# PINTO0309/human-instance-segmentation

Measured on AMD Instinct MI355X. Metric: ROI-masks/sec (fwd) + train step/s, B0 640×480×8-ROI, 1/2/4/8 MI355X, higher is better.
Workload: dtype bf16; 1 GPU; C2: B0 inference 640x480, batch 32/GPU x 8 ROIs/img, ROI 64x48, mask 128x96; global_batch=32, parallelism=dp1 (images sharded, model replicated, no collective), schedule=2-stream pipeline (UNet of step k+1 overlaps head of step k)

## Files before the change

human-instance-segmentation_amd/csrc/misc.hip:

```cpp
#include <float.h>
#include "common.h"
#include "gfx950_prims.h"
#include "head2.h"

namespace hiseg {

static inline unsigned nblocks(long long n, int bs) { return (unsigned)((n + bs - 1) / bs); }

template <typename T>
__global__ void __launch_bounds__(256) maxpool2x2_kernel(const void* in, int N, int H, int W, int C, void* out) {
  constexpr int K = Chunk<T>::N;
  const int nch = C / K;
  const int Ho = H / 2, Wo = W / 2;
  const long long gid = (long long)blockIdx.x * 256 + threadIdx.x;
  const long long total = (long long)N * Ho * Wo * nch;
  if (gid >= total) return;
  const int ch = (int)(gid % nch);
  long long p = gid / nch;
  const int x = (int)(p % Wo); p /= Wo;
  const int y = (int)(p % Ho);
  const int n = (int)(p / Ho);
  const uint4* src = reinterpret_cast<const uint4*>(in);
  float m[K], v[K];
  for (int e = 0; e < K; ++e) m[e] = -FLT_MAX;
#pragma unroll
  for (int dy = 0; dy < 2; ++dy)
#pragma unroll
    for (int dx = 0; dx < 2; ++dx) {
      const long long pix = ((long long)n * H + 2 * y + dy) * W + 2 * x + dx;
      Chunk<T>::unpack(src[pix * nch + ch], v);
#pragma unroll
      for (int e = 0; e < K; ++e) m[e] = fmaxf(m[e], v[e]);
    }
  reinterpret_cast<uint4*>(out)[gid] = Chunk<T>::pack(m);
}
// ... 276 lines not shown
  if (v2) hipLaunchKernelGGL(se_gate_out_kernel<true>, g2, dim3(256), lds, s, partial, splits, C, b1, Cr, act, beta, w2, b2, gate);
  else hipLaunchKernelGGL(se_gate_out_kernel<false>, g2, dim3(256), lds, s, partial, splits, C, b1, Cr, act, beta, w2, b2, gate);
}

static bool se2_enabled() {
  const char* e = getenv("HISEG_SE2");
  return !(e && atoi(e) == 0);
}

static void se_mlp(const float* w1, const float* b1, int Cr, const float* w2, const float* b2, int act, float beta, int N,
                   int HW, int C, float* scratch, float* gate, hipStream_t s) {
  hipLaunchKernelGGL(se_hidden_kernel, dim3(N, (Cr + 3) / 4), dim3(256), 0, s, gate, HW, C, w1, b1, Cr, act, beta, scratch);
  hipLaunchKernelGGL(se_out_kernel, dim3(N, (C + 3) / 4), dim3(256), 0, s, scratch, C, Cr, w2, b2, gate);
}

template <typename T>
__global__ void __launch_bounds__(256) channel_scale_kernel(const void* x, int N, long long HW, int C, const float* gate,
                                                            void* out) {
  constexpr int K = Chunk<T>::N;
  const int nch = C / K;
  const long long gid = (long long)blockIdx.x * 256 + threadIdx.x;
  const long long total = (long long)N * HW * nch;
  if (gid >= total) return;
  const int ch = (int)(gid % nch);
  const long long n = gid / nch / HW;
  float v[K];
  Chunk<T>::unpack(reinterpret_cast<const uint4*>(x)[gid], v);
  const float* g = gate + n * C + ch * K;
#pragma unroll
  for (int e = 0; e < K; ++e) v[e] *= g[e];
  reinterpret_cast<uint4*>(out)[gid] = Chunk<T>::pack(v);
}

constexpr int kDwXS = 4;

template <typename T, int KS, int ST>
__global__ void __launch_bounds__(256) dwconv_kernel(const void* in, int H, int W, int C, const float* w,
                                                     const float* scale, const float* shift, int act, void* out,
                                                     int Ho, int Wo, float* gap) {
  constexpr int V = Chunk<T>::N;
  constexpr int NIN = (kDwXS - 1) * ST + KS;
  __shared__ float red[256 * V];
  const int nch = C / V;
  const int g0 = blockIdx.z * 256;
  const int CT = (nch - g0) < 256 ? (nch - g0) : 256;
  const int R = 256 / CT;
  const int t = threadIdx.x;
  const int cl = t % CT, r = t / CT;
  const int ch = g0 + cl;
  const bool live = r < R;
  const int n = blockIdx.y, tiles = gridDim.x, tile = blockIdx.x;
  const int sx = (Wo + kDwXS - 1) / kDwXS;
  const int strips = Ho * sx;
  const int s0 = (int)((long long)strips * tile / tiles), s1 = (int)((long long)strips * (tile + 1) / tiles);
  const int c = ch * V;
  const int pad = KS / 2;
  float sc[V], sh[V], gs[V];
#pragma unroll
  for (int e = 0; e < V; ++e) { sc[e] = scale[c + e]; sh[e] = shift[c + e]; gs[e] = 0.f; }
  const uint4* src = reinterpret_cast<const uint4*>(in) + (long long)n * H * W * nch;
  uint4* dst = reinterpret_cast<uint4*>(out) + (long long)n * Ho * Wo * nch;
  if (live) {
    for (int st = s0 + r; st < s1; st += R) {
      const int oy = st / sx;
      const int ox0 = (st - oy * sx) * kDwXS;
      float acc[kDwXS][V];
#pragma unroll
// ... 137 lines not shown
            if (kx < 0 || kx >= KS) continue;
#pragma unroll
            for (int e = 0; e < 4; ++e) acc[xo][e] += wk[ky * KS + kx][e] * v[e];
          }
        }
      }
#pragma unroll
      for (int xo = 0; xo < kDwXS; ++xo) {
        if (ox0 + xo >= Wo) break;
        float o[4];
#pragma unroll
        for (int e = 0; e < 4; ++e) {
          o[e] = apply_act(acc[xo][e] * sc[e] + sh[e], act);
          gs[e] += o[e];
        }
        dst[((long long)oy * Wo + ox0 + xo) * nq + q] = make_uint2(f2bf2(o[0], o[1]), f2bf2(o[2], o[3]));
      }
    }
  }
  if (gap == nullptr) return;
#pragma unroll
  for (int e = 0; e < 4; ++e) red[t * 4 + e] = gs[e];
  __syncthreads();
  if (r == 0 && live) {
    for (int rr = 1; rr < R; ++rr)
#pragma unroll
      for (int e = 0; e < 4; ++e) gs[e] += red[(rr * CT + cl) * 4 + e];
    float* gp = gap + ((long long)n * tiles + tile) * C + c;
#pragma unroll
    for (int e = 0; e < 4; ++e) gp[e] = gs[e];
  }
}

constexpr int kDwTH = 8, kDwTW = 16, kDwCG = 64, kDwPS = kDwCG * 2 + 8;
template <int KS, int ST, bool ZP = false, int CP = 4>
__global__ void __launch_bounds__(256) dwconv_t_kernel(const void* in, int H, int W, int C, const float* w,
                                                       const float* scale, const float* shift, int act, void* out,
                                                       int Ho, int Wo, float* gap, int xcd) {
  constexpr int IH = (kDwTH - 1) * ST + KS, IW = (kDwTW - 1) * ST + KS;
  constexpr int NIN = (kDwXS - 1) * ST + KS;
  constexpr int NSTRIP = kDwTH * (kDwTW / kDwXS);
  extern __shared__ __attribute__((aligned(16))) char dws[];
  const int t = threadIdx.x;
  int bt = blockIdx.x, n = blockIdx.y, gz = blockIdx.z;
  if (xcd) {
    const int nwg = gridDim.x * gridDim.y * gridDim.z;
    const int orig = blockIdx.x + gridDim.x * (blockIdx.y + gridDim.y * blockIdx.z);
    int wg = xcd_major(orig, nwg);
    if (xcd == 2) {
      gz = wg % gridDim.z;
      wg /= gridDim.z;
      bt = wg % gridDim.x;
      n = wg / gridDim.x;
    } else {
      bt = wg % gridDim.x;
      wg /= gridDim.x;
      n = wg % gridDim.y;
      gz = wg / gridDim.y;
    }
  }
  const int g0 = gz * kDwCG;
  const int ntx = (Wo + kDwTW - 1) / kDwTW;
  const int ty = bt / ntx, tx = bt - ty * ntx;
  const int oy0 = ty * kDwTH, ox0 = tx * kDwTW;
  const int iy0 = oy0 * ST - KS / 2, ix0 = ox0 * ST - KS / 2;
  const int nch = C >> 3;
  const uint4* src = reinterpret_cast<const uint4*>(in) + (long long)n * H * W * nch;
// ... 499 lines not shown
}

extern "C" int hiseg_dw_gap_tiles(int N, int Ho, int Wo) {
  const int strips = Ho * ((Wo + kDwXS - 1) / kDwXS);
  int t = 2048 / (N > 0 ? N : 1);
  if (t < 1) t = 1;
  int by_len = strips / 2;
  if (by_len < 1) by_len = 1;
  return t < by_len ? t : by_len;
}

static bool dw_q_enabled() {
  const char* e = getenv("HISEG_DWCONV_Q");
  return !(e && atoi(e) == 0);
}

static bool dw_use_tiles(int dtype, int C, int K, int stride) {
  const char* e = getenv("HISEG_DWCONV_T");
  const int m = e ? atoi(e) : 1;
  if (dtype != HISEG_BF16 || m == 0 || !dw_q_enabled()) return false;
  return m == 2 || (C < 2048 && ((stride == 1 && C >= 64) || (K == 5 && C >= 192)));
}

extern "C" int hiseg_dw_gap_parts(int dtype, int N, int Ho, int Wo, int C, int K, int stride) {
  if (dw_use_tiles(dtype, C, K, stride)) return ((Ho + kDwTH - 1) / kDwTH) * ((Wo + kDwTW - 1) / kDwTW);
  return hiseg_dw_gap_tiles(N, Ho, Wo);
}

static size_t dw_lds(int KS, int ST) {
  const size_t win = (size_t)((kDwTH - 1) * ST + KS) * ((kDwTW - 1) * ST + KS) * kDwPS;
  return win > 256 * 4 * sizeof(float) ? win : 256 * 4 * sizeof(float);
}

static int dw_xcd_remap() {
  const char* e = getenv("HISEG_DWCONV_XCD");
  return e ? atoi(e) : 2;
}

static bool dw_zero_pad_q(int K, int stride) {
  const char* e = getenv("HISEG_DWCONV_QZP");
  return !(e && e[0] == '0') && (K == 3 || stride == 2);
}

static int dw_xcd_remap_q() {
  const char* e = getenv("HISEG_DWCONV_QXCD");
  return e ? atoi(e) : 2;
}

template <int KS, int ST>
static void dw_t_attr() {
  static bool done = false;
  if (!done) {
    (void)hipFuncSetAttribute((const void*)dwconv_t_kernel<KS, ST, false>, hipFuncAttributeMaxDynamicSharedMemorySize,
                              (int)dw_lds(KS, ST));
    (void)hipFuncSetAttribute((const void*)dwconv_t_kernel<KS, ST, true>, hipFuncAttributeMaxDynamicSharedMemorySize,
                              (int)dw_lds(KS, ST));
    (void)hipFuncSetAttribute((const void*)dwconv_t_kernel<KS, ST, false, 2>,
                              hipFuncAttributeMaxDynamicSharedMemorySize, (int)dw_lds(KS, ST));
    (void)hipFuncSetAttribute((const void*)dwconv_t_kernel<KS, ST, true, 2>, hipFuncAttributeMaxDynamicSharedMemorySize,
                              (int)dw_lds(KS, ST));
    done = true;
  }
}

static bool dw_zero_pad(int K) {
  const char* e = getenv("HISEG_DWCONV_ZP");
  const int m = e ? atoi(e) : 2;
  return m == 2 || (K == 3 && m == 1);
}

static int dw_cp(int K, int C) {
  const char* e = getenv("HISEG_DWCONV_CP");
  const int m = e ? atoi(e) : 0;
  return m == 2 || m == 4 ? m : (K == 5 || C < 512 ? 2 : 4);
}

static int dwconv_launch(int dtype, const void* in, int N, int H, int W, int C, int K, int stride, const float* w,
                         const float* scale, const float* shift, int act, void* out, int Ho, int Wo, float* gap,
                         hipStream_t s) {
  HISEG_REQUIRE(in && w && scale && shift && out && N > 0 && H > 0 && W > 0, HISEG_ERR_BAD_ARG, "dwconv: bad args");
  HISEG_REQUIRE(act != HISEG_ACT_SWISH, HISEG_ERR_BAD_ARG, "dwconv: Swish(beta) is not an EfficientNet activation");
  HISEG_REQUIRE(C % chunk_of(dtype) == 0, HISEG_ERR_BAD_SHAPE, "dwconv: C must be chunk aligned");
  HISEG_REQUIRE((K == 3 || K == 5) && (stride == 1 || stride == 2), HISEG_ERR_BAD_SHAPE, "dwconv: K %d stride %d", K,
                stride);
  HISEG_REQUIRE(Ho == (H + 2 * (K / 2) - K) / stride + 1 && Wo == (W + 2 * (K / 2) - K) / stride + 1, HISEG_ERR_BAD_SHAPE,
                "dwconv: output grid mismatch");
  HISEG_REQUIRE((reinterpret_cast<uintptr_t>(w) & 15) == 0 && (long long)H * W * C < (1ll << 31), HISEG_ERR_BAD_SHAPE,
                "dwconv: weights must be 16-B aligned, image < 2^31 elements");
  const int nch = C / chunk_of(dtype);
  const int nq = C / 4, ctq = dw_quads_per_block(nq);
  const int tiles = hiseg_dw_gap_tiles(N, Ho, Wo);
  dim3 grid(tiles, N, (nch + 255) / 256);
  dim3 gridq(tiles, N, (nq + ctq - 1) / ctq);
  const bool dwq = dw_q_enabled();
  const bool dwt = dw_use_tiles(dtype, C, K, stride);
  const int tiles2 = ((Ho + kDwTH - 1) / kDwTH) * ((Wo + kDwTW - 1) / kDwTW);
  const dim3 gridt(tiles2, N, (C + kDwCG - 1) / kDwCG);
#define DW_L(KS, ST)                                                                                          \
  do {                                                                                                        \
    if (dtype == HISEG_BF16 && dwt) {                                                                         \
      dw_t_attr<KS, ST>();                                                                                    \
      const bool zp = dw_zero_pad(KS), cp2 = dw_cp(KS, C) == 2;                                                    \
      if (zp && cp2)                                                                                          \
        hipLaunchKernelGGL((dwconv_t_kernel<KS, ST, true, 2>), gridt, dim3(256), dw_lds(KS, ST), s, in, H, W, \
// ... 268 lines not shown
```

human-instance-segmentation_amd/hiseg/_lib.py:

```python
from __future__ import annotations

import contextlib
import ctypes
import os

import torch

_HERE = os.path.dirname(os.path.abspath(__file__))
LIB_PATH = os.environ.get("HISEG_LIB", os.path.join(_HERE, "libhiseg.so"))

HISEG_F32 = 0
HISEG_BF16 = 1
HISEG_POST_F32, HISEG_POST_F16, HISEG_POST_F32_TO_F16 = 0, 2, 3
ACT_NONE, ACT_RELU, ACT_SIGMOID, ACT_SILU, ACT_GELU, ACT_SWISH = 0, 1, 2, 3, 4, 5


class ActCode(int):

    def __new__(cls, code: int, beta: float = 1.0):
        o = int.__new__(cls, code)
        o.beta = float(beta)
        return o

    def __repr__(self):
# ... 235 lines not shown
        "hiseg_xcd_major": ([c_int, c_int], c_int),
        "hiseg_xcd_major_fill": ([c_int, c_int, c_int, P], c_int),
        "hiseg_stream_create_cu_mask": ([ctypes.POINTER(ctypes.c_uint), c_int, ctypes.POINTER(c_void_p)], c_int),
        "hiseg_stream_destroy": ([P], c_int),
        "hiseg_comm_load": ([ctypes.c_char_p], c_int),
        "hiseg_comm_unique_id": ([P], c_int),
        "hiseg_comm_init": ([ctypes.POINTER(c_void_p), c_int, P, c_int, c_int], c_int),
        "hiseg_comm_all_reduce": ([P, P, c_ll, c_int, c_int, P], c_int),
        "hiseg_comm_destroy": ([P], c_int),
        "hiseg_roi_align_fwd": ([ctypes.POINTER(RoiAlignDesc), P], c_int),
        "hiseg_conv2d_fwd": ([ctypes.POINTER(Conv2dDesc), P], c_int),
        "hiseg_conv2d_fwd_variant": ([ctypes.POINTER(Conv2dDesc), c_int, P], c_int),
        "hiseg_conv2d_workspace_bytes": ([ctypes.POINTER(Conv2dDesc)], c_ll),
        "hiseg_conv2d_last_path": ([], c_int),
        "hiseg_conv2d_path_stats": ([ctypes.POINTER(c_ll), c_int, c_int], c_int),
        "hiseg_maxpool2x2_fwd": ([c_int, P, c_int, c_int, c_int, c_int, P, P], c_int),
        "hiseg_attn_spatial_fwd": ([c_int, P, c_int, c_int, c_int, c_int, P, c_int, P, P, P, P], c_int),
        "hiseg_attn_map_fwd": ([c_int, P, c_int, c_int, c_int, c_int, P, c_int, P, P, P], c_int),
        "hiseg_pixel_scale_fwd": ([c_int, P, c_ll, c_int, P, P, P], c_int),
        "hiseg_conv2d_fused_ok": ([ctypes.POINTER(Conv2dDesc)], c_int),
        "hiseg_resblock_fused_ok": ([ctypes.POINTER(Conv2dDesc), ctypes.POINTER(Conv2dDesc)], c_int),
        "hiseg_resblock_fwd": ([ctypes.POINTER(Conv2dDesc), ctypes.POINTER(Conv2dDesc), P], c_int),
        "hiseg_hier_combine_tn_fwd": ([P, c_int, c_int, c_int, P, P, P, P, c_int, c_float, c_int, P, P, P, P, P, P],
                                      c_int),
        "hiseg_gap_splits": ([c_int], c_int),
        "hiseg_se_gate_fwd": ([c_int, P, c_int, c_int, c_int, P, P, c_int, P, P, c_int, c_float, P, P, P], c_int),
        "hiseg_channel_scale_fwd": ([c_int, P, c_int, c_int, c_int, P, P, P], c_int),
        "hiseg_dwconv_fwd": ([c_int, P, c_int, c_int, c_int, c_int, c_int, c_int, P, P, P, c_int, P,
                              c_int, c_int, P], c_int),
        "hiseg_dw_gap_tiles": ([c_int, c_int, c_int], c_int),
        "hiseg_dw_gap_parts": ([c_int, c_int, c_int, c_int, c_int, c_int, c_int], c_int),
        "hiseg_dwconv_gap_fwd": ([c_int, P, c_int, c_int, c_int, c_int, c_int, c_int, P, P, P, c_int, P,
                                  c_int, c_int, P, P], c_int),
        "hiseg_se_gate_partials_fwd": ([P, c_int, c_int, c_int, c_int, P, P, c_int, P, P, c_int, P, P], c_int),
        "hiseg_image_max_fwd": ([P, c_ll, P, P], c_int),
        "hiseg_input_norm_fwd": ([c_int, P, c_int, c_int, c_int, c_int, P, P, P, P, c_int, P], c_int),
        "hiseg_hier_combine_fwd": ([c_int, P, c_int, c_int, c_int, P, c_int, P, P, P, c_int, c_float, c_int, P, P,
                                    P, P, P, P, P, P], c_int),
        "hiseg_ubf_ln_tables": ([P, c_int, c_int, c_int, P, P, P, P, c_float, c_int, P, P, P, P, P], c_int),
        "hiseg_nhwc_to_nchw_fwd": ([c_int, P, c_int, c_int, c_int, c_int, c_int, c_int, P, P], c_int),
        "hiseg_nchw_to_nhwc_fwd": ([c_int, P, c_int, c_int, c_int, c_int, P, c_int, P], c_int),
        "hiseg_instance_masks_fwd": ([P, c_int, c_int, c_int, c_int, P, P], c_int),
        "hiseg_binary_masks_fwd": ([c_int, P, c_int, c_int, c_int, c_int, P, P, P, P], c_int),
        "hiseg_resize_bilinear_fwd": ([P, c_int, c_int, c_int, P, c_int, c_int, P], c_int),
        "hiseg_distance_mask_fwd": ([P, c_ll, P, P, P], c_int),
        "hiseg_output_conv_fwd": ([P, c_int, c_int, c_int, P, P, P, P], c_int),
        "hiseg_conv2d_wgrad_dims": ([ctypes.POINTER(Conv2dDesc), c_int, P, P, P], c_int),
        "hiseg_conv2d_wgrad": ([ctypes.POINTER(Conv2dDesc), P, c_int, c_int, c_int, P, c_int, P], c_int),
        "hiseg_wgrad_path_stats": ([ctypes.POINTER(c_ll), c_int], c_int),
        "hiseg_struct_sizes": ([ctypes.POINTER(c_ll), c_int], c_int),
        "hiseg_conv2d_stats_tiles": ([ctypes.POINTER(Conv2dDesc)], c_int),
        "hiseg_bn_finalize_n": ([P, c_int, c_int, c_ll, P, P, c_float, c_float, P, P, P, P, P, P, P], c_int),
        "hiseg_wgrad_last_path": ([], c_int),
        "hiseg_conv2d_wgrad_reduce": ([P, c_int, ctypes.POINTER(WgradMap), P, P, c_int, P], c_int),
        "hiseg_pack_weights": ([P, c_int, c_int, P], c_int),
        "hiseg_bn_partials": ([], c_int),
        "hiseg_bn_last_path": ([], c_int),
        "hiseg_bn_stats": ([c_int, P, c_ll, c_int, c_int, c_int, P, P], c_int),
        "hiseg_bn_finalize": ([P, c_int, c_ll, P, P, c_float, c_float, P, P, P, P, P, P, P], c_int),
        "hiseg_bn_apply": ([ctypes.POINTER(BnApplyDesc), P], c_int),
        "hiseg_bn_bwd": ([ctypes.POINTER(BnBwdDesc), P], c_int),
        "hiseg_dropout2d_mask": ([c_int, c_int, c_float, ctypes.c_ulonglong, P, P], c_int),
        "hiseg_dropout2d_mask_dev": ([c_int, c_int, c_float, P, ctypes.c_ulonglong, P, P], c_int),
        "hiseg_seed_advance": ([P, P], c_int),
        "hiseg_relu_bwd": ([c_int, c_ll, c_int, c_int, EwView, EwView, P, EwView, P], c_int),
        "hiseg_sigmoid_bwd": ([c_int, c_ll, c_int, EwView, EwView, EwView, P], c_int),
# ... 207 lines not shown
```

human-instance-segmentation_amd/hiseg/engine.py:

```python
from __future__ import annotations

from typing import Dict, Optional, Tuple

import torch
import torch.nn as nn

from . import _lib as L
from . import ops
from .effunet import DepthwiseSeparableConv, InvertedResidual
from .layers import LayerNorm2d, Swish
from .ops import Act, round_up

ACT_NONE, ACT_RELU, ACT_SIGMOID, ACT_SILU = L.ACT_NONE, L.ACT_RELU, L.ACT_SIGMOID, L.ACT_SILU
ACT_GELU, ACT_SWISH = L.ACT_GELU, L.ACT_SWISH


def act_code(m: nn.Module) -> int:
    if isinstance(m, nn.ReLU):
        return ACT_RELU
    if isinstance(m, nn.SiLU):
        return ACT_SILU
    if isinstance(m, Swish):
        return ACT_SILU if float(m.beta) == 1.0 else L.ActCode(ACT_SWISH, float(m.beta))
    if isinstance(m, nn.GELU):
# ... 364 lines not shown
    out, edges = ops.boundary_blend(em, R, E.f32(mod.blend_weight, (1,)), want_edges)
    return (out, edges) if want_edges else out


def _resize(x: torch.Tensor, H: int, W: int, lib) -> torch.Tensor:
    N, C, h, w = x.shape
    if (h, w) == (H, W):
        return x
    out = torch.empty(N, C, H, W, dtype=torch.float32, device=x.device)
    L.check(lib.hiseg_resize_bilinear_fwd(x.data_ptr(), N * C, h, w, out.data_ptr(), H, W, L.stream_ptr()),
            "resize_bilinear")
    return out


def _se(E: Ctx, se: nn.Module, h: Act) -> torch.Tensor:
    rd, c = se.conv_reduce.out_channels, se.conv_reduce.in_channels
    return ops.se_gate(h, E.f32(se.conv_reduce.weight, (rd, c)), E.f32(se.conv_reduce.bias),
                       E.f32(se.conv_expand.weight, (c, rd)), E.f32(se.conv_expand.bias), ACT_SILU)


def _dw(E: Ctx, conv: nn.Conv2d, bn, x: Act, act: int) -> Act:
    w, s, h, k, stride = E.dw(conv, bn)
    return ops.dwconv(x, w, s, h, k, stride, act)


def _dw_se(E: Ctx, conv: nn.Conv2d, bn, se: nn.Module, x: Act) -> Tuple[Act, torch.Tensor]:
    w, s, h, k, stride = E.dw(conv, bn)
    rd, c = se.conv_reduce.out_channels, se.conv_reduce.in_channels
    return ops.dwconv_se_gate(x, w, s, h, k, stride, ACT_SILU, E.f32(se.conv_reduce.weight, (rd, c)),
                              E.f32(se.conv_reduce.bias), E.f32(se.conv_expand.weight, (c, rd)),
                              E.f32(se.conv_expand.bias), ACT_SILU)


def mbconv(E: Ctx, blk: nn.Module, x: Act, out_cpad: Optional[int] = None) -> Act:
    if isinstance(blk, DepthwiseSeparableConv):
        h, g = _dw_se(E, blk.conv_dw, blk.bn1, blk.se, x)
        return ops.conv2d(E.conv(blk.conv_pw, blk.bn2), h, in_scale=g, residual=x if blk.has_skip else None,
                          out_cpad=out_cpad)
    if isinstance(blk, InvertedResidual):
        h = ops.conv2d(E.conv(blk.conv_pw, blk.bn1, ACT_SILU), x)
        h, g = _dw_se(E, blk.conv_dw, blk.bn2, blk.se, h)
        return ops.conv2d(E.conv(blk.conv_pwl, blk.bn3), h, in_scale=g, residual=x if blk.has_skip else None,
                          out_cpad=out_cpad)
    raise TypeError(type(blk))


def _block_out_channels(blk: nn.Module) -> int:
    return (blk.conv_pw if isinstance(blk, DepthwiseSeparableConv) else blk.conv_pwl).out_channels


def _drain(gen):
    while True:
        try:
            next(gen)
        except StopIteration as e:
            return e.value


def unet_logit(E: Ctx, pre: nn.Module, images: torch.Tensor) -> torch.Tensor:
    return _drain(unet_logit_iter(E, pre, images))


def unet_logit_iter(E: Ctx, pre: nn.Module, images: torch.Tensor):
    B, _, H, W = images.shape
    if H % 32 or W % 32:
        raise NotImplementedError(f"image size {H}x{W} must be a multiple of 32 for the EfficientNet-UNet")
    x = ops.input_norm(images, E.f32(pre.norm_mean, (3,)), E.f32(pre.norm_std, (3,)), E.dtype)
    return (yield from effunet_forward_iter(E, pre.model, x))


def effunet_forward(E: Ctx, net: nn.Module, x: Act) -> torch.Tensor:
    return _drain(effunet_forward_iter(E, net, x))


# ... 197 lines not shown
```

human-instance-segmentation_amd/hiseg/ops.py:

```python
from __future__ import annotations

import ctypes
from dataclasses import dataclass
from typing import Optional

import torch

from . import _lib as L

_TORCH_TO_HISEG = {torch.float32: L.HISEG_F32, torch.bfloat16: L.HISEG_BF16}


def chunk_elems(dtype: torch.dtype) -> int:
    return 8 if dtype == torch.bfloat16 else 4


def round_up(x: int, m: int) -> int:
    return (x + m - 1) // m * m


def hdtype(dtype: torch.dtype) -> int:
    try:
        return _TORCH_TO_HISEG[dtype]
    except KeyError:
# ... 451 lines not shown

def dwconv(x: Act, w: torch.Tensor, scale: torch.Tensor, shift: torch.Tensor, k: int, stride: int, act: int) -> Act:
    assert x.coff == 0 and x.cstride == x.C
    pad = k // 2
    Ho = (x.H + 2 * pad - k) // stride + 1
    Wo = (x.W + 2 * pad - k) // stride + 1
    out = Act.new(x.N, Ho, Wo, x.C, x.dtype, x.t.device, zero=False)
    L.check(L.lib().hiseg_dwconv_fwd(hdtype(x.dtype), x.ptr(), x.N, x.H, x.W, x.C, k, stride, w.data_ptr(),
                                     scale.data_ptr(), shift.data_ptr(), act, out.ptr(), Ho, Wo, L.stream_ptr()),
            "dwconv")
    return out


def dwconv_se_gate(x: Act, w: torch.Tensor, scale: torch.Tensor, shift: torch.Tensor, k: int, stride: int, act: int,
                   w1, b1, w2, b2, se_act: int):
    assert x.coff == 0 and x.cstride == x.C
    pad = k // 2
    Ho = (x.H + 2 * pad - k) // stride + 1
    Wo = (x.W + 2 * pad - k) // stride + 1
    lib = L.lib()
    out = Act.new(x.N, Ho, Wo, x.C, x.dtype, x.t.device, zero=False)
    tiles = lib.hiseg_dw_gap_parts(hdtype(x.dtype), x.N, Ho, Wo, x.C, k, stride)
    partial = torch.empty(x.N * tiles * x.C, dtype=torch.float32, device=x.t.device)
    L.check(lib.hiseg_dwconv_gap_fwd(hdtype(x.dtype), x.ptr(), x.N, x.H, x.W, x.C, k, stride, w.data_ptr(),
                                     scale.data_ptr(), shift.data_ptr(), act, out.ptr(), Ho, Wo, partial.data_ptr(),
                                     L.stream_ptr()), "dwconv_gap")
    gate = torch.empty(x.N, x.C, dtype=torch.float32, device=x.t.device)
    L.check(lib.hiseg_se_gate_partials_fwd(partial.data_ptr(), tiles, x.N, Ho * Wo, x.C, w1.data_ptr(), _ptr(b1),
                                           w1.shape[0], w2.data_ptr(), _ptr(b2), se_act, gate.data_ptr(),
                                           L.stream_ptr()), "se_gate_partials")
    return out, gate


def input_norm(images: torch.Tensor, mean: torch.Tensor, std: torch.Tensor, dtype: torch.dtype) -> Act:
    _require_gpu(images)
    x = images.contiguous().float()
    B, C, H, W = x.shape
    lib = L.lib()
    maxbuf = torch.empty(1, dtype=torch.float32, device=x.device)
    L.check(lib.hiseg_image_max_fwd(x.data_ptr(), x.numel(), maxbuf.data_ptr(), L.stream_ptr()), "image_max")
    out = Act.new(B, H, W, C, dtype, x.device, zero=False)
    L.check(lib.hiseg_input_norm_fwd(hdtype(dtype), x.data_ptr(), B, C, H, W, maxbuf.data_ptr(), mean.data_ptr(),
                                     std.data_ptr(), out.ptr(), out.cstride, L.stream_ptr()), "input_norm")
    return out


def hier_combine(low: torch.Tensor, N: int, h: int, w: int, tfeat: Optional[Act], ut_w, ut_scale, ut_shift, ut_act,
                 u1_w, u1_b, t_w, t_b, want_aux: bool, per_sample: bool = False, tn2: Optional[torch.Tensor] = None):
    dev = low.device
    logits = torch.empty(N, 3, 2 * h, 2 * w, dtype=torch.float32, device=dev)
    bgfg = torch.empty(N, 2, 2 * h, 2 * w, dtype=torch.float32, device=dev) if want_aux else None
    tn = torch.empty(N, 2, 2 * h, 2 * w, dtype=torch.float32, device=dev) if want_aux else None
    if tn2 is not None:
        assert tn2.dtype == torch.float32 and tn2.is_contiguous() and tn2.numel() == N * 4 * h * w * 2
        L.check(L.lib().hiseg_hier_combine_tn_fwd(low.data_ptr(), N, h, w, tn2.data_ptr(), ut_w.data_ptr(),
                                                  ut_scale.data_ptr(), ut_shift.data_ptr(), int(ut_act),
                                                  L.act_beta(ut_act), int(per_sample), u1_w.data_ptr(), u1_b.data_ptr(),
                                                  logits.data_ptr(), _ptr(bgfg), _ptr(tn), L.stream_ptr()),
                "hier_combine_tn")
        return logits, bgfg, tn
    assert tfeat.coff == 0 and tfeat.cstride == tfeat.C and (tfeat.H, tfeat.W) == (2 * h, 2 * w)
    L.check(L.lib().hiseg_hier_combine_fwd(hdtype(tfeat.dtype), low.data_ptr(), N, h, w, tfeat.ptr(), tfeat.C,
                                           ut_w.data_ptr(), ut_scale.data_ptr(), ut_shift.data_ptr(), int(ut_act),
                                           L.act_beta(ut_act), int(per_sample), u1_w.data_ptr(), u1_b.data_ptr(), t_w.data_ptr(), t_b.data_ptr(),
                                           logits.data_ptr(), _ptr(bgfg), _ptr(tn), L.stream_ptr()), "hier_combine")
    return logits, bgfg, tn
# ... 520 lines not shown
```

include/hiseg.h:

```cpp
#ifndef HISEG_H_
#define HISEG_H_

#ifdef __cplusplus
extern "C" {
#endif

typedef void* hiseg_stream_t;

enum hiseg_dtype { HISEG_F32 = 0, HISEG_BF16 = 1 };

enum hiseg_act { HISEG_ACT_NONE = 0, HISEG_ACT_RELU = 1, HISEG_ACT_SIGMOID = 2, HISEG_ACT_SILU = 3,
                 HISEG_ACT_GELU = 4, HISEG_ACT_SWISH = 5 };

enum hiseg_status {
  HISEG_OK = 0,
  HISEG_ERR_BAD_ARG = -1,
  HISEG_ERR_BAD_SHAPE = -2,
  HISEG_ERR_BAD_DTYPE = -3,
  HISEG_ERR_LAUNCH = -4
};

int hiseg_version(void);
const char* hiseg_last_error_string(void);
int hiseg_built_for_gfx950(void);
// ... 62 lines not shown
#define HISEG_CONV_PATH_SMALL 9
#define HISEG_CONV_PATH_ROWS 10
#define HISEG_CONV_PATH_RESBLOCK 11
#define HISEG_CONV_PATH_FAMILIES 12
int hiseg_conv2d_last_path(void);
int hiseg_conv2d_path_stats(long long* counts, int n, int reset);

int hiseg_maxpool2x2_fwd(int dtype, const void* in, int N, int H, int W, int C, void* out,
                         hiseg_stream_t stream);

int hiseg_attn_spatial_fwd(int dtype, const void* x, int N, int H, int W, int C, const float* w7,
                           int k, float* stats, float* att, void* out, hiseg_stream_t stream);
int hiseg_attn_map_fwd(int dtype, const void* x, int N, int H, int W, int C, const float* w7,
                       int k, float* stats, float* att, hiseg_stream_t stream);
int hiseg_pixel_scale_fwd(int dtype, const void* x, long long P, int C, const float* att, void* out,
                          hiseg_stream_t stream);

int hiseg_gap_splits(int HW);
int hiseg_se_gate_fwd(int dtype, const void* x, int N, int HW, int C, const float* w1,
                      const float* b1, int Cr, const float* w2, const float* b2, int act, float act_beta,
                      float* partial, float* gate, hiseg_stream_t stream);

int hiseg_channel_scale_fwd(int dtype, const void* x, int N, int HW, int C, const float* gate,
                            void* out, hiseg_stream_t stream);

int hiseg_dwconv_fwd(int dtype, const void* in, int N, int H, int W, int C, int K, int stride,
                     const float* w, const float* scale, const float* shift, int act, void* out,
                     int Ho, int Wo, hiseg_stream_t stream);
int hiseg_dw_gap_tiles(int N, int Ho, int Wo);
int hiseg_dw_gap_parts(int dtype, int N, int Ho, int Wo, int C, int K, int stride);
int hiseg_dwconv_gap_fwd(int dtype, const void* in, int N, int H, int W, int C, int K, int stride,
                         const float* w, const float* scale, const float* shift, int act, void* out,
                         int Ho, int Wo, float* gap_partial, hiseg_stream_t stream);
int hiseg_se_gate_partials_fwd(float* partial, int splits, int N, int HW, int C, const float* w1,
                               const float* b1, int Cr, const float* w2, const float* b2, int act,
                               float* gate, hiseg_stream_t stream);

int hiseg_image_max_fwd(const float* x, long long n, float* maxbuf, hiseg_stream_t stream);
int hiseg_input_norm_fwd(int dtype, const float* x, int B, int C, int H, int W, const float* maxbuf,
                         const float* mean, const float* std, void* out, int cpad,
                         hiseg_stream_t stream);

int hiseg_hier_combine_fwd(int dtype, const float* low, int N, int h, int w, const void* tfeat,
                           int Ct, const float* ut_w, const float* ut_scale, const float* ut_shift,
                           int ut_act, float ut_beta, int ut_per_sample, const float* u1_w,
                           const float* u1_b, const float* t_w, const float* t_b, float* logits,
                           float* bgfg, float* tn, hiseg_stream_t stream);
int hiseg_hier_combine_tn_fwd(const float* low, int N, int h, int w, const float* tn2, const float* ut_w,
                              const float* ut_scale, const float* ut_shift, int ut_act, float ut_beta,
                              int ut_per_sample, const float* u1_w, const float* u1_b, float* logits,
                              float* bgfg, float* tn, hiseg_stream_t stream);
int hiseg_ubf_ln_tables(const float* low, int N, int h, int w, const float* ut_w, const float* ut_b,
                        const float* gamma, const float* beta, float eps, int fold_bias, float* mean,
                        float* invstd, float* scale, float* shift, hiseg_stream_t stream);

int hiseg_nhwc_to_nchw_fwd(int dtype, const void* in, int N, int H, int W, int C, int cstride,
                           int coff, float* out, hiseg_stream_t stream);
int hiseg_nchw_to_nhwc_fwd(int dtype, const float* in, int N, int C, int H, int W, void* out,
                           int cpad, hiseg_stream_t stream);

int hiseg_instance_masks_fwd(const float* logits, int N, int mh, int mw, int dilation,
                             float* instance, hiseg_stream_t stream);
int hiseg_binary_masks_fwd(int dtype, const void* u, int u_cstride, int B, int H, int W,
                           const float* oc_w, const float* oc_b, float* binary,
                           hiseg_stream_t stream);

// ... 14 lines not shown
```

Before: 17020 ROI-masks/s.

## Fuse MBConv 1x1 expand conv into depthwise conv tile kernel

Adds a kernel that computes the 1x1 expansion (MFMA bf16 with BN+SiLU) directly into the LDS halo tile of the depthwise conv, then runs the depthwise conv, BN, activation and SE GAP partials from that tile. This avoids writing the expanded activation to global memory and reading it back, for small-input-channel inference blocks. The cost is recomputing the expansion on halo pixels. It is limited to a whitelist of layer shapes (Ca 16/24/40) and falls back to the old path otherwise.

```diff
diff --git a/human-instance-segmentation_amd/csrc/dwconv_tile.h b/human-instance-segmentation_amd/csrc/dwconv_tile.h
--- /dev/null
+++ b/human-instance-segmentation_amd/csrc/dwconv_tile.h
@@ -0,0 +1,14 @@
+#pragma once
+
+namespace hiseg {
+
+constexpr int kDwXS = 4;
+constexpr int kDwTH = 8, kDwTW = 16;
+constexpr int kDwCG = 64;
+constexpr int kDwPS = kDwCG * 2 + 8;
+
+int dw_cp(int K, int C);
+bool dw_zero_pad(int K);
+int dw_xcd_remap();
+
+}
diff --git a/human-instance-segmentation_amd/csrc/mbconv_fused.hip b/human-instance-segmentation_amd/csrc/mbconv_fused.hip
--- /dev/null
+++ b/human-instance-segmentation_amd/csrc/mbconv_fused.hip
@@ -0,0 +1,273 @@
+#include "common.h"
+#include "gfx950_prims.h"
+#include "dwconv_tile.h"
+
+namespace hiseg {
+
+struct MbconvArgs {
+  const void* x; int x_cstride, x_coff, Ca;
+  const void* ew; int ew_rows, K_pad;
+  const float* escale; const float* eshift;
+  int N, H, W, C;
+  const float* w; const float* scale; const float* shift; int act;
+  void* out; int Ho, Wo; float* gap; int xcd;
+};
+
+template <int KS, int ST, int NKS>
+__global__ void __launch_bounds__(256) mbconv_dw_kernel(MbconvArgs a) {
+  constexpr int IH = (kDwTH - 1) * ST + KS, IW = (kDwTW - 1) * ST + KS;
+  constexpr int NIN = (kDwXS - 1) * ST + KS;
+  constexpr int NSTRIP = kDwTH * (kDwTW / kDwXS);
+  constexpr int NPIX = IH * IW, NGRP = (NPIX + 15) / 16;
+  constexpr int CP = 2;
+  extern __shared__ __attribute__((aligned(16))) char dws[];
+  const int t = threadIdx.x;
+  const int H = a.H, W = a.W, C = a.C, Ho = a.Ho, Wo = a.Wo;
+  int bt = blockIdx.x, n = blockIdx.y, gz = blockIdx.z;
+  if (a.xcd) {
+    const int nwg = gridDim.x * gridDim.y * gridDim.z;
+    const int orig = blockIdx.x + gridDim.x * (blockIdx.y + gridDim.y * blockIdx.z);
+    int wg = xcd_major(orig, nwg);
+    if (a.xcd == 2) {
+      gz = wg % gridDim.z;
+      wg /= gridDim.z;
+      bt = wg % gridDim.x;
+      n = wg / gridDim.x;
+    } else {
+      bt = wg % gridDim.x;
+      wg /= gridDim.x;
+      n = wg % gridDim.y;
+      gz = wg / gridDim.y;
+    }
+  }
+  const int g0 = gz * kDwCG;
+  const int ntx = (Wo + kDwTW - 1) / kDwTW;
+  const int ty = bt / ntx, tx = bt - ty * ntx;
+  const int oy0 = ty * kDwTH, ox0 = tx * kDwTW;
+  const int iy0 = oy0 * ST - KS / 2, ix0 = ox0 * ST - KS / 2;
+
+  {
+    const int lane = t & 63, wv = t >> 6;
+    const int g = lane >> 4, pl = lane & 15;
+    const __amdgpu_buffer_rsrc_t rW = buf_rsrc(a.ew, (unsigned)((long long)a.ew_rows * a.K_pad * 2));
+    const __amdgpu_buffer_rsrc_t rX = buf_rsrc(a.x, (unsigned)((long long)a.N * H * W * a.x_cstride * 2));
+    uint4 af[4][NKS];
+#pragma unroll
+    for (int i = 0; i < 4; ++i)
+#pragma unroll
+      for (int ks = 0; ks < NKS; ++ks) {
+        const int row = g0 + 16 * i + pl;
+        const unsigned off = row < a.ew_rows ? (unsigned)((row * a.K_pad + 32 * ks + 8 * g) * 2) : kOobOffset;
+        const u32x4 v = __builtin_amdgcn_raw_buffer_load_b128(rW, off, 0, 0);
+        af[i][ks] = make_uint4(v.x, v.y, v.z, v.w);
+      }
+    floatx4 sc[4], sh[4];
+#pragma unroll
+    for (int i = 0; i < 4; ++i)
+#pragma unroll
+      for (int e = 0; e < 4; ++e) {
+        const int col = g0 + 16 * i + 4 * g + e;
+        sc[i][e] = a.escale[col < C ? col : 0];
+        sh[i][e] = a.eshift[col < C ? col : 0];
+      }
+    const int img = n * H * W;
+    constexpr int UB = 4;
+#pragma unroll 1
+    for (int gb = wv; gb < NGRP; gb += 4 * UB) {
+      uint4 bf[UB][NKS];
+      bool inimg[UB];
+#pragma unroll
+      for (int u = 0; u < UB; ++u) {
+        const int pix = (gb + 4 * u) * 16 + pl;
+        const int hy = pix / IW, hx = pix - hy * IW;
+        const int iy = iy0 + hy, ix = ix0 + hx;
+        inimg[u] = pix < NPIX && (unsigned)iy < (unsigned)H && (unsigned)ix < (unsigned)W;
+#pragma unroll
+        for (int ks = 0; ks < NKS; ++ks) {
+          const unsigned off = inimg[u] && 32 * ks + 8 * g < a.Ca
+              ? (unsigned)(((img + iy * W + ix) * a.x_cstride + a.x_coff + 32 * ks + 8 * g) * 2) : kOobOffset;
+          const u32x4 v = __builtin_amdgcn_raw_buffer_load_b128(rX, off, 0, 0);
+          bf[u][ks] = make_uint4(v.x, v.y, v.z, v.w);
+        }
+      }
+#pragma unroll
+      for (int u = 0; u < UB; ++u) {
+        if (gb + 4 * u >= NGRP) break;
+        const int pix = (gb + 4 * u) * 16 + pl;
+        floatx4 acc[4];
+#pragma unroll
+        for (int i = 0; i < 4; ++i) acc[i] = floatx4{0.f, 0.f, 0.f, 0.f};
+#pragma unroll
+        for (int ks = 0; ks < NKS; ++ks)
+#pragma unroll
+          for (int i = 0; i < 4; ++i)
+            acc[i] = __builtin_amdgcn_mfma_f32_16x16x32_bf16(__builtin_bit_cast(bf16x8_t, af[i][ks]),
+                                                             __builtin_bit_cast(bf16x8_t, bf[u][ks]), acc[i], 0, 0, 0);
+#pragma unroll
+        for (int i = 0; i < 4; ++i) {
+          float v[4];
+#pragma unroll
+          for (int e = 0; e < 4; ++e) {
+            v[e] = acc[i][e] * sc[i][e] + sh[i][e];
+            v[e] = apply_act(v[e], HISEG_ACT_SILU);
+          }
+          uint2 q = make_uint2(f2bf2(v[0], v[1]), f2bf2(v[2], v[3]));
+          if (!inimg[u] || g0 + 16 * i + 4 * g >= C) q = make_uint2(0u, 0u);
+          if (pix < NPIX) *reinterpret_cast<uint2*>(dws + pix * kDwPS + (16 * i + 4 * g) * 2) = q;
+        }
+      }
+    }
+  }
+
+  constexpr int NQ = kDwCG / CP, NG = 256 / NQ;
+  const int qd = t % NQ, it = t / NQ;
+  const int c = g0 + qd * CP;
+  const bool live = c < C;
+  const int cc = live ? c : 0;
+  typedef float f2v __attribute__((ext_vector_type(2)));
+  float sc[CP], sh[CP], gs[CP];
+  f2v wp[KS * KS];
+#pragma unroll
+  for (int k = 0; k < KS * KS; ++k) {
+    const float2 q = *reinterpret_cast<const float2*>(a.w + k * C + cc);
+    wp[k] = f2v{q.x, q.y};
+  }
+#pragma unroll
+  for (int e = 0; e < CP; ++e) { sc[e] = a.scale[cc + e]; sh[e] = a.shift[cc + e]; gs[e] = 0.f; }
+#pragma unroll
+  for (int k = 0; k < KS * KS; ++k) asm volatile("" : "+v"(wp[k]));
+  __syncthreads();
+  unsigned* dst = reinterpret_cast<unsigned*>(a.out) + (long long)n * Ho * Wo * (C >> 1);
+#pragma unroll
+  for (int sj = 0; sj < NSTRIP / NG; ++sj) {
+    const int st = it + NG * sj;
+    const int ry = st / (kDwTW / kDwXS), rx = (st - ry * (kDwTW / kDwXS)) * kDwXS;
+    const int oy = oy0 + ry, ox = ox0 + rx;
+    if (!live || oy >= Ho) continue;
+    f2v a2[kDwXS];
+#pragma unroll
+    for (int xo = 0; xo < kDwXS; ++xo) a2[xo] = f2v{0.f, 0.f};
+#pragma unroll
+    for (int ky = 0; ky < KS; ++ky) {
+      const char* row = dws + ((ry * ST + ky) * IW + rx * ST) * kDwPS + qd * 2 * CP;
+#pragma unroll
+      for (int j = 0; j < NIN; ++j) {
+        const unsigned raw = *reinterpret_cast<const unsigned*>(row + j * kDwPS);
+        const f2v v = f2v{__uint_as_float(raw << 16), __uint_as_float(raw & 0xffff0000u)};
+#pragma unroll
+        for (int xo = 0; xo < kDwXS; ++xo) {
+          const int kx = j - xo * ST;
+          if (kx < 0 || kx >= KS) continue;
+          a2[xo] = __builtin_elementwise_fma(wp[ky * KS + kx], v, a2[xo]);
+        }
+      }
+    }
+#pragma unroll
+    for (int xo = 0; xo < kDwXS; ++xo) {
+      if (ox + xo >= Wo) break;
+      float o[CP];
+#pragma unroll
+      for (int e = 0; e < CP; ++e) {
+        o[e] = apply_act(a2[xo][e] * sc[e] + sh[e], a.act);
+        gs[e] += o[e];
+      }
+      dst[((long long)oy * Wo + ox + xo) * (C >> 1) + (c >> 1)] = f2bf2(o[0], o[1]);
+    }
+  }
+  if (a.gap == nullptr) return;
+  __syncthreads();
+  float* red = reinterpret_cast<float*>(dws);
+#pragma unroll
+  for (int e = 0; e < CP; ++e) red[t * CP + e] = gs[e];
+  __syncthreads();
+  if (it == 0 && live) {
+    for (int r = 1; r < NG; ++r)
+#pragma unroll
+      for (int e = 0; e < CP; ++e) gs[e] += red[(r * NQ + qd) * CP + e];
+    float* gp = a.gap + ((long long)n * gridDim.x + bt) * C + c;
+#pragma unroll
+    for (int e = 0; e < CP; ++e) gp[e] = gs[e];
+  }
+}
+
+}
+
+using namespace hiseg;
+
+static size_t mb_lds(int KS, int ST) {
+  const size_t win = (size_t)((kDwTH - 1) * ST + KS) * ((kDwTW - 1) * ST + KS) * kDwPS;
+  return win > 256 * 2 * sizeof(float) ? win : 256 * 2 * sizeof(float);
+}
+
+static bool mb_measured_faster(int Ca, int C, int K, int stride) {
+  if (K != 3) return false;
+  if (stride == 2) return (Ca == 16 && C == 96) || (Ca == 40 && C == 240);
+  return Ca == 24 && C == 144;
+}
+
+extern "C" int hiseg_mbconv_fused_ok(const hiseg_conv2d_desc* e, int C, int K, int stride, int dw_act, int training,
+                                     int any_form) {
+  if (!e || training) return 0;
+  if (e->dtype != HISEG_BF16 || e->out_dtype != HISEG_BF16) return 0;
+  if (e->act != HISEG_ACT_SILU || dw_act != HISEG_ACT_SILU) return 0;
+  if (e->KH != 1 || e->KW != 1 || e->stride != 1 || e->pad != 0 || e->a_up != 1 || e->convT) return 0;
+  if (e->srcB || e->Cb || e->in_scale || e->residual || e->mul || e->out2 || e->px_scale || e->head2_out || e->a_gate ||
+      e->res_gate || e->stats_partial || e->bnb_partial || e->workspace)
+    return 0;
+  if ((K != 3 && K != 5) || (stride != 1 && stride != 2)) return 0;
+  if (e->Cout != C || C % 8 || e->Ca <= 0 || e->Ca % 8 || e->Ca > 64) return 0;
+  if (e->Cout_pad < C || e->K_pad < (e->Ca + 31) / 32 * 32) return 0;
+  if (!e->srcA || !e->weight || !e->scale || !e->shift || e->N <= 0 || e->H <= 0 || e->W <= 0) return 0;
+  if ((e->a_cstride | e->a_coff) & 7 || ((uintptr_t)e->srcA & 15) || ((uintptr_t)e->weight & 15)) return 0;
+  if (e->Ho != e->H || e->Wo != e->W) return 0;
+  const int Ho = (e->H + 2 * (K / 2) - K) / stride + 1, Wo = (e->W + 2 * (K / 2) - K) / stride + 1;
+  const long long lim = 0x7fffffffll, px = (long long)e->N * e->H * e->W;
+  if (px * e->a_cstride * 2 >= lim || px * C * 2 >= lim || (long long)e->N * Ho * Wo * C * 2 >= lim ||
+      (long long)e->Cout_pad * e->K_pad * 2 >= lim)
+    return 0;
+  if (!dw_zero_pad(K) || dw_cp(K, C) != 2) return 0;
+  if (!any_form && !mb_measured_faster(e->Ca, C, K, stride)) return 0;
+  return ((Ho + kDwTH - 1) / kDwTH) * ((Wo + kDwTW - 1) / kDwTW);
+}
+
+template <int KS, int ST>
+static void mb_launch(const MbconvArgs& a, int nks, dim3 grid, hipStream_t s) {
+  static bool done = false;
+  if (!done) {
+    (void)hipFuncSetAttribute((const void*)mbconv_dw_kernel<KS, ST, 1>, hipFuncAttributeMaxDynamicSharedMemorySize,
+                              (int)mb_lds(KS, ST));
+    (void)hipFuncSetAttribute((const void*)mbconv_dw_kernel<KS, ST, 2>, hipFuncAttributeMaxDynamicSharedMemorySize,
+                              (int)mb_lds(KS, ST));
+    done = true;
+  }
+  if (nks == 1) hipLaunchKernelGGL((mbconv_dw_kernel<KS, ST, 1>), grid, dim3(256), mb_lds(KS, ST), s, a);
+  else hipLaunchKernelGGL((mbconv_dw_kernel<KS, ST, 2>), grid, dim3(256), mb_lds(KS, ST), s, a);
+}
+
+extern "C" int hiseg_mbconv_expand_dw_fwd(const hiseg_conv2d_desc* e, int C, int K, int stride, const float* w,
+                                          const float* scale, const float* shift, int act, void* out, int Ho, int Wo,
+                                          float* gap_partial, hiseg_stream_t stream) {
+  HISEG_REQUIRE(e && w && scale && shift && out && gap_partial, HISEG_ERR_BAD_ARG, "mbconv_expand_dw: bad args");
+  HISEG_REQUIRE(hiseg_mbconv_fused_ok(e, C, K, stride, act, 0, 1) > 0, HISEG_ERR_BAD_ARG,
+                "mbconv_expand_dw: the kernel does not take this layer (ask hiseg_mbconv_fused_ok first)");
+  HISEG_REQUIRE(Ho == (e->H + 2 * (K / 2) - K) / stride + 1 && Wo == (e->W + 2 * (K / 2) - K) / stride + 1,
+                HISEG_ERR_BAD_SHAPE, "mbconv_expand_dw: output grid mismatch");
+  HISEG_REQUIRE((reinterpret_cast<uintptr_t>(w) & 15) == 0, HISEG_ERR_BAD_SHAPE,
+                "mbconv_expand_dw: depthwise weights must be 16-B aligned");
+  MbconvArgs a;
+  a.x = e->srcA; a.x_cstride = e->a_cstride; a.x_coff = e->a_coff; a.Ca = e->Ca;
+  a.ew = e->weight; a.ew_rows = e->Cout_pad; a.K_pad = e->K_pad;
+  a.escale = e->scale; a.eshift = e->shift;
+  a.N = e->N; a.H = e->H; a.W = e->W; a.C = C;
+  a.w = w; a.scale = scale; a.shift = shift; a.act = act;
+  a.out = out; a.Ho = Ho; a.Wo = Wo; a.gap = gap_partial; a.xcd = dw_xcd_remap();
+  const int tiles = ((Ho + kDwTH - 1) / kDwTH) * ((Wo + kDwTW - 1) / kDwTW);
+  const dim3 grid(tiles, e->N, (C + kDwCG - 1) / kDwCG);
+  const int nks = (e->Ca + 31) / 32;
+  hipStream_t s = (hipStream_t)stream;
+  if (K == 3 && stride == 1) mb_launch<3, 1>(a, nks, grid, s);
+  else if (K == 3) mb_launch<3, 2>(a, nks, grid, s);
+  else if (stride == 1) mb_launch<5, 1>(a, nks, grid, s);
+  else mb_launch<5, 2>(a, nks, grid, s);
+  return hiseg_check_launch("mbconv_expand_dw");
+}
diff --git a/human-instance-segmentation_amd/csrc/misc.hip b/human-instance-segmentation_amd/csrc/misc.hip
--- a/human-instance-segmentation_amd/csrc/misc.hip
+++ b/human-instance-segmentation_amd/csrc/misc.hip
@@ -1,6 +1,7 @@
 #include <float.h>
 #include "common.h"
 #include "gfx950_prims.h"
+#include "dwconv_tile.h"
 #include "head2.h"
 
 namespace hiseg {
@@ -343,7 +344,6 @@
   reinterpret_cast<uint4*>(out)[gid] = Chunk<T>::pack(v);
 }
 
-constexpr int kDwXS = 4;
 
 template <typename T, int KS, int ST>
 __global__ void __launch_bounds__(256) dwconv_kernel(const void* in, int H, int W, int C, const float* w,
@@ -547,7 +547,6 @@
   }
 }
 
-constexpr int kDwTH = 8, kDwTW = 16, kDwCG = 64, kDwPS = kDwCG * 2 + 8;
 template <int KS, int ST, bool ZP = false, int CP = 4>
 __global__ void __launch_bounds__(256) dwconv_t_kernel(const void* in, int H, int W, int C, const float* w,
                                                        const float* scale, const float* shift, int act, void* out,
@@ -1113,7 +1112,7 @@
   return win > 256 * 4 * sizeof(float) ? win : 256 * 4 * sizeof(float);
 }
 
-static int dw_xcd_remap() {
+int hiseg::dw_xcd_remap() {
   const char* e = getenv("HISEG_DWCONV_XCD");
   return e ? atoi(e) : 2;
 }
@@ -1144,13 +1143,13 @@
   }
 }
 
-static bool dw_zero_pad(int K) {
+bool hiseg::dw_zero_pad(int K) {
   const char* e = getenv("HISEG_DWCONV_ZP");
   const int m = e ? atoi(e) : 2;
   return m == 2 || (K == 3 && m == 1);
 }
 
-static int dw_cp(int K, int C) {
+int hiseg::dw_cp(int K, int C) {
   const char* e = getenv("HISEG_DWCONV_CP");
   const int m = e ? atoi(e) : 0;
   return m == 2 || m == 4 ? m : (K == 5 || C < 512 ? 2 : 4);
diff --git a/human-instance-segmentation_amd/hiseg/_lib.py b/human-instance-segmentation_amd/hiseg/_lib.py
--- a/human-instance-segmentation_amd/hiseg/_lib.py
+++ b/human-instance-segmentation_amd/hiseg/_lib.py
@@ -291,6 +291,9 @@
         "hiseg_dw_gap_parts": ([c_int, c_int, c_int, c_int, c_int, c_int, c_int], c_int),
         "hiseg_dwconv_gap_fwd": ([c_int, P, c_int, c_int, c_int, c_int, c_int, c_int, P, P, P, c_int, P,
                                   c_int, c_int, P, P], c_int),
+        "hiseg_mbconv_fused_ok": ([ctypes.POINTER(Conv2dDesc), c_int, c_int, c_int, c_int, c_int, c_int], c_int),
+        "hiseg_mbconv_expand_dw_fwd": ([ctypes.POINTER(Conv2dDesc), c_int, c_int, c_int, P, P, P, c_int, P, c_int,
+                                        c_int, P, P], c_int),
         "hiseg_se_gate_partials_fwd": ([P, c_int, c_int, c_int, c_int, P, P, c_int, P, P, c_int, P, P], c_int),
         "hiseg_image_max_fwd": ([P, c_ll, P, P], c_int),
         "hiseg_input_norm_fwd": ([c_int, P, c_int, c_int, c_int, c_int, P, P, P, P, c_int, P], c_int),
diff --git a/human-instance-segmentation_amd/hiseg/engine.py b/human-instance-segmentation_amd/hiseg/engine.py
--- a/human-instance-segmentation_amd/hiseg/engine.py
+++ b/human-instance-segmentation_amd/hiseg/engine.py
@@ -420,14 +420,35 @@
                               E.f32(se.conv_expand.bias), ACT_SILU)
 
 
+MBCONV_FUSED = True
+
+
+def _expand_dw_se(E: Ctx, blk: nn.Module, x: Act) -> Optional[Tuple[Act, torch.Tensor]]:
+    if blk.training or x.dtype != torch.bfloat16:
+        return None
+    p = E.conv(blk.conv_pw, blk.bn1, ACT_SILU)
+    k, stride = blk.conv_dw.kernel_size[0], blk.conv_dw.stride[0]
+    if not ops.mbconv_fused_parts(p, x, k, stride, ACT_SILU):
+        return None
+    w, s, h, k, stride = E.dw(blk.conv_dw, blk.bn2)
+    se = blk.se
+    rd, c = se.conv_reduce.out_channels, se.conv_reduce.in_channels
+    return ops.mbconv_expand_dw_se_gate(p, x, w, s, h, k, stride, ACT_SILU, E.f32(se.conv_reduce.weight, (rd, c)),
+                                        E.f32(se.conv_reduce.bias), E.f32(se.conv_expand.weight, (c, rd)),
+                                        E.f32(se.conv_expand.bias), ACT_SILU)
+
+
 def mbconv(E: Ctx, blk: nn.Module, x: Act, out_cpad: Optional[int] = None) -> Act:
     if isinstance(blk, DepthwiseSeparableConv):
         h, g = _dw_se(E, blk.conv_dw, blk.bn1, blk.se, x)
         return ops.conv2d(E.conv(blk.conv_pw, blk.bn2), h, in_scale=g, residual=x if blk.has_skip else None,
                           out_cpad=out_cpad)
     if isinstance(blk, InvertedResidual):
-        h = ops.conv2d(E.conv(blk.conv_pw, blk.bn1, ACT_SILU), x)
-        h, g = _dw_se(E, blk.conv_dw, blk.bn2, blk.se, h)
+        hg = _expand_dw_se(E, blk, x) if MBCONV_FUSED else None
+        if hg is None:
+            h = ops.conv2d(E.conv(blk.conv_pw, blk.bn1, ACT_SILU), x)
+            hg = _dw_se(E, blk.conv_dw, blk.bn2, blk.se, h)
+        h, g = hg
         return ops.conv2d(E.conv(blk.conv_pwl, blk.bn3), h, in_scale=g, residual=x if blk.has_skip else None,
                           out_cpad=out_cpad)
     raise TypeError(type(blk))
diff --git a/human-instance-segmentation_amd/hiseg/ops.py b/human-instance-segmentation_amd/hiseg/ops.py
--- a/human-instance-segmentation_amd/hiseg/ops.py
+++ b/human-instance-segmentation_amd/hiseg/ops.py
@@ -507,6 +507,48 @@
     return out, gate
 
 
+def mbconv_fused_parts(p: ConvPlan, x: Act, k: int, stride: int, act: int, training: bool = False,
+                       any_form: bool = False) -> int:
+    if p.convT or x.dtype != torch.bfloat16 or x.C > p.ca:
+        return 0
+    d = _conv_desc(p, x, None, None, None, None, out_dtype=x.dtype)
+    return int(L.lib().hiseg_mbconv_fused_ok(ctypes.byref(d), p.cout, k, stride, int(act), int(training),
+                                             int(any_form)))
+
+
+def mbconv_expand_dw(p: ConvPlan, x: Act, w: torch.Tensor, scale: torch.Tensor, shift: torch.Tensor, k: int,
+                     stride: int, act: int, any_form: bool = False):
+    if RECORD is not None or GATE is not None:
+        return None
+    parts = mbconv_fused_parts(p, x, k, stride, act, any_form=any_form)
+    if parts <= 0:
+        return None
+    C = p.cout
+    pad = k // 2
+    Ho = (x.H + 2 * pad - k) // stride + 1
+    Wo = (x.W + 2 * pad - k) // stride + 1
+    out = Act.new(x.N, Ho, Wo, C, x.dtype, x.t.device, zero=False)
+    partial = torch.empty(x.N * parts * C, dtype=torch.float32, device=x.t.device)
+    d = _conv_desc(p, x, None, None, None, None, out_dtype=x.dtype)
+    L.check(L.lib().hiseg_mbconv_expand_dw_fwd(ctypes.byref(d), C, k, stride, w.data_ptr(), scale.data_ptr(),
+                                               shift.data_ptr(), int(act), out.ptr(), Ho, Wo, partial.data_ptr(),
+                                               L.stream_ptr()), "mbconv_expand_dw")
+    return out, partial, parts
+
+
+def mbconv_expand_dw_se_gate(p: ConvPlan, x: Act, w: torch.Tensor, scale: torch.Tensor, shift: torch.Tensor, k: int,
+                             stride: int, act: int, w1, b1, w2, b2, se_act: int, any_form: bool = False):
+    r = mbconv_expand_dw(p, x, w, scale, shift, k, stride, act, any_form=any_form)
+    if r is None:
+        return None
+    out, partial, parts = r
+    gate = torch.empty(x.N, out.C, dtype=torch.float32, device=x.t.device)
+    L.check(L.lib().hiseg_se_gate_partials_fwd(partial.data_ptr(), parts, x.N, out.H * out.W, out.C, w1.data_ptr(),
+                                               _ptr(b1), w1.shape[0], w2.data_ptr(), _ptr(b2), se_act,
+                                               gate.data_ptr(), L.stream_ptr()), "se_gate_partials")
+    return out, gate
+
+
 def input_norm(images: torch.Tensor, mean: torch.Tensor, std: torch.Tensor, dtype: torch.dtype) -> Act:
     _require_gpu(images)
     x = images.contiguous().float()
diff --git a/include/hiseg.h b/include/hiseg.h
--- a/include/hiseg.h
+++ b/include/hiseg.h
@@ -118,6 +118,11 @@
 int hiseg_dwconv_gap_fwd(int dtype, const void* in, int N, int H, int W, int C, int K, int stride,
                          const float* w, const float* scale, const float* shift, int act, void* out,
                          int Ho, int Wo, float* gap_partial, hiseg_stream_t stream);
+int hiseg_mbconv_fused_ok(const hiseg_conv2d_desc* expand, int C, int K, int stride, int dw_act, int training,
+                          int any_form);
+int hiseg_mbconv_expand_dw_fwd(const hiseg_conv2d_desc* expand, int C, int K, int stride, const float* w,
+                               const float* scale, const float* shift, int act, void* out, int Ho, int Wo,
+                               float* gap_partial, hiseg_stream_t stream);
 int hiseg_se_gate_partials_fwd(float* partial, int splits, int N, int HW, int C, const float* w1,
                                const float* b1, int Cr, const float* w2, const float* b2, int act,
                                float* gate, hiseg_stream_t stream);
```

New measurement: 17110 ROI-masks/s (median of 6 runs). No clear change (+0.5%).
